# mitschabaude/montgomery

Hardware: AMD Instinct MI355X
Metric: BLS12-377 G1 MSM throughput (higher is better)
Workload: dtype u32

## Files before the change

### montgomery_amd/csrc/msm_internal.h

```cpp
#pragma once
#include "kernel_inst.h"
#include "sort_kernels.h"
#include "tree_kernels.h"
#include "te_kernels.h"
#include "narrow_kernels.h"
#include "host_field.h"
#include "scalar_vec.h"
#include "../../include/msm_hip.h"

#include <algorithm>
#include <cstdarg>
#include <cstdio>
#include <cstring>
#include <atomic>
#include <chrono>
#include <condition_variable>
#include <exception>
#include <functional>
#include <memory>
#include <mutex>
#include <string>
#include <system_error>
#include <thread>
#include <vector>

#ifdef MSM_TUNING
#define MSM_KNOB(var, name, lo) do { if (const char* _e = getenv(name)) var = std::max<long long>((lo), atoll(_e)); } while (0)
#define MSM_KNOB_SET(name) (getenv(name) != nullptr)
#else
#define MSM_KNOB(var, name, lo) do { } while (0)
#define MSM_KNOB_SET(name) false
#endif

namespace msmi {

struct DevBuf {
  void* p = nullptr;
  size_t cap = 0;
};

// ... 112 lines not shown
      std::function<void()> job = std::move(job_);
      job_ = nullptr;
      l.unlock();
      std::exception_ptr e;
      try { job(); } catch (...) { e = std::current_exception(); }
      l.lock();
      err_ = e;
      busy_ = false;
      cv_.notify_all();
    }
  }
  std::mutex mu_;
  std::condition_variable cv_;
  std::function<void()> job_;
  std::exception_ptr err_;
  bool busy_ = false, quit_ = false;
  std::thread th_;
};

}

struct msm_ctx {
  std::unique_ptr<msmi::HelperThread> helper;
  int curve = 0;
  int device = 0;
  hipStream_t stream = nullptr;
  hipEvent_t ev[12] = {};
  hipEvent_t ev_dig[2] = {};
  std::string err;
  int n_cu = 256;

  struct WindowTables {
    int c = 0, K = 0;
    uint64_t lo = 0, n = 0;
    bool in_rows = false;
    msmi::DevBuf buf;
    bool covers(uint64_t l, uint64_t m) const { return K && lo == l && n == m; }
    bool whole_set_pinned() const { return K && in_rows; }
    void clear() { c = K = 0; lo = n = 0; in_rows = false; }
    void drop(msm_ctx* ctx) { clear(); ctx->release(buf); }
  };
  struct PointSet {
    msmi::DevBuf rows;
    uint64_t n = 0;
    bool live = false;
    WindowTables tab;
    const uint32_t* table_rows() const { return (const uint32_t*)(tab.in_rows ? rows.p : tab.buf.p); }
    void release(msm_ctx* ctx) { tab.drop(ctx); ctx->release(rows); *this = PointSet(); }
  };
  std::vector<PointSet> sets = std::vector<PointSet>(1);
  int cur_set = 0;
  PointSet& pts() { return sets[cur_set]; }
  const PointSet& pts() const { return sets[cur_set]; }
  uint32_t* reset_points(uint64_t n) { return reset_points(pts(), n); }
  uint32_t* reset_points(PointSet& s, uint64_t n) {
    s.n = 0;
    s.tab.drop(this);
    cand_n = 0;
    ensure(s.rows, std::max<uint64_t>(n, 1) * row_words() * 4);
    return (uint32_t*)s.rows.p;
  }
  uint64_t cand_lo = 0, cand_n = 0;
  int cand_c = 0;
  uint64_t tables_limit = 0;
  std::vector<void*> allocs;
  std::vector<msm_ctx*> children;
  std::vector<std::unique_ptr<msmi::HelperThread>> fan;

  msmi::DevBuf scal, errflag, misc;
  uint32_t* h_info = nullptr;
  static constexpr int STAGE_THREADS = 4, STAGE_SLOTS = 2;
  static constexpr size_t STAGE_CHUNK = (size_t)16 << 20;
  char* stage_pin = nullptr;
  bool staging_ready = false;
  hipStream_t stage_stream[STAGE_THREADS] = {};
  hipEvent_t stage_ev[STAGE_THREADS][STAGE_SLOTS + 1] = {};
  static constexpr int MAX_PIECES = 6;
  hipEvent_t piece_ev[MAX_PIECES][STAGE_THREADS] = {};
  uint64_t ws_budget = 0;
  uint64_t ws_limit = 0;

  struct Workspace {
    msmi::DevBuf dig, counts, cursor, tail_off, info, slots, block_hist, scan_partial, desc, columns2, rows_sum, bucket_proj, bufA, bufB,
        scratch, columns, partials, part, dig2, idx2, rec, blk_tab2, slots2, dest, rows1, parts, sub;
    hipStream_t stream = nullptr;
    hipStream_t side = nullptr;
    hipEvent_t ev[8] = {};
    uint32_t* h_info = nullptr;
    uint32_t* h_part = nullptr;
    msmi::DevBuf* all[27] = {&dig, &counts, &cursor, &tail_off, &info, &slots, &block_hist, &scan_partial, &desc, &columns2, &rows_sum,
                       &bucket_proj, &bufA, &bufB, &scratch, &columns, &partials, &part, &dig2, &idx2, &rec, &blk_tab2, &slots2, &dest, &rows1,
                       &parts, &sub};
  };
  static constexpr int N_WS = 2;
  Workspace ws[N_WS];

  msm_host::Curve6 hc;
  msm_host::Fe6 k_dev_to_host;
  msm_host::TeCurve6 hte;
  msm_host::Fe6 k_te_to_host;
  bool is_te() const { return curve == MSM_CURVE_ED_ON_BLS12_377; }
  int nl() const { return msmi::curve_info(curve).nl; }
  int nw() const { return msmi::curve_info(curve).nw; }
  size_t coord_bytes() const { return (size_t)nw() * 4; }
  uint64_t row_words() const { return is_te() ? (uint64_t)msm::te::TE_ROW_WORDS : (uint64_t)msm::ROW_WORDS; }
  int sum_words() const { return is_te() ? msmi::TE_SUM_WORDS : msmi::W_SUM_WORDS; }

  void ensure(msmi::DevBuf& b, size_t bytes) {
    if (bytes <= b.cap) return;
    if (b.p) HIPCHK(hipFree(b.p));
    b.p = nullptr;
    b.cap = 0;
    size_t want = bytes + bytes / 16 + 256;
    const hipError_t e = hipMalloc(&b.p, want);
    if (e != hipSuccess) {
      (void)hipGetLastError();
      b.p = nullptr;
      throw msmi::HipFail{e, "hipMalloc(&b.p, want)", __LINE__, __FILE__};
    }
    b.cap = want;
  }
  void release(msmi::DevBuf& b) {
    if (b.p) (void)hipFree(b.p);
    b.p = nullptr;
    b.cap = 0;
  }
};

// ... 22 lines not shown

#define ROWS_TO_PLANES(ctx, ...)                                                                       \
  do {                                                                                                 \
    if ((ctx)->nw() == 8) hipLaunchKernelGGL((k_test_rows_to_planes<8>), __VA_ARGS__);                 \
    else hipLaunchKernelGGL((k_test_rows_to_planes<12>), __VA_ARGS__);                                 \
  } while (0)

namespace msmi {
using namespace msm;

int fail(msm_ctx* ctx, int code, const char* fmt, ...);
int fail_hip(msm_ctx* ctx, const HipFail& f);

inline uint64_t point_lo(const msm_opts* opts) { return opts ? opts->point_lo : 0; }
int check_points(msm_ctx* ctx, uint64_t n, const msm_opts* opts, int code, const char* who, bool empty_ok = true);

#define MSM_CATCH_ALL(ctx)                                                                                  \
  catch (const HipFail& f) { return fail_hip(ctx, f); }                                                     \
  catch (const MsmFail& f) { return fail(ctx, f.code, "%s", f.msg.c_str()); }                               \
  catch (const std::bad_alloc&) { return fail(ctx, MSM_ERR_INTERNAL, "host memory allocation failed"); }    \
  catch (const std::exception& e) { return fail(ctx, MSM_ERR_INTERNAL, "unexpected exception: %s", e.what()); } \
  catch (...) { return fail(ctx, MSM_ERR_INTERNAL, "unexpected exception"); }

int pick_window(bool te, uint64_t n, int glv_max_bits);

struct Plan {
  int c, K, L_log;
  int bits = 0;
  bool fold = false;
  uint32_t L;
  bool no_glv;
  bool strict = false;
  bool lone = false;
  uint32_t b_lo = 0, b_n = 0xFFFFFFFFu;
  uint32_t bt_lo = 0, bt_n = 0xFFFFFFFFu;
  bool tables = false;
  const uint32_t* tab_rows = nullptr;
  uint64_t tab_lo = 0, tab_n = 0;
  bool merged = false;
  int batch = 0;
  BatchScalars batch_sc{};
  struct Narrow {
    int width = 0;
    uint64_t first = 0;
    NarrowFmt fmt{};
    const NarrowBatchScalars* nb = nullptr;
  } nar;
  const uint32_t* idx = nullptr;
};

int make_plan(const msm_ctx* ctx, uint64_t n, const msm_opts* opts, Plan& pl, bool for_tables = false, int narrow_bits = 0);
int pick_window_narrow(bool te, uint64_t n, int bits, bool one_level = false);
int make_run_plan(msm_ctx* ctx, uint64_t n, const msm_opts* opts, bool placed, Plan& pl, bool& tables_wanted, bool note_range = false);

struct GroupStats {
  uint64_t n_pairs = 0;
  uint64_t n_pairs_algo = 0;
  uint64_t max_bucket = 0;
  int rounds = 0;
  float ms_digits = 0, ms_sort = 0, ms_acc = 0, ms_red = 0, ms_r1 = 0;
  GroupStats& operator+=(const GroupStats& o) {
    n_pairs += o.n_pairs;
    n_pairs_algo += o.n_pairs_algo;
    max_bucket = std::max(max_bucket, o.max_bucket);
    rounds += o.rounds;
    ms_digits += o.ms_digits; ms_sort += o.ms_sort; ms_acc += o.ms_acc; ms_red += o.ms_red; ms_r1 += o.ms_r1;
    return *this;
  }
};

struct RoundGeom {
  uint32_t steps, grid;
  uint64_t T;
};

RoundGeom round_geom(const msm_ctx* ctx, uint64_t n_out, bool gather = false, bool lone = false);
void release_workspaces(msm_ctx* ctx);
long double window_bytes(const msm_ctx* ctx, uint64_t n, const Plan& pl);
int windows_per_group(const msm_ctx* ctx, uint64_t n, const Plan& pl);
uint64_t point_pieces(const msm_ctx* ctx, uint64_t n, const Plan& pl);

void words_to_fe6(msm_host::Fe6& r, const uint32_t* w, int nw = 12);
void fe6_to_bytes(uint8_t* out, const msm_host::Fe6& a);
void device_coord_to_wire(const msm_host::Field6& F, const msm_host::Fe6& k_to_host, const uint32_t* w, int nw, uint8_t* out);
void plane_element_to_wire(const msm_ctx* ctx, const uint32_t* planes, uint64_t cap, uint64_t e, uint8_t* out_xy);
void reduce_buckets(msm_ctx* ctx, msm_ctx::Workspace& w, const uint4* fin, uint64_t fin_cap, const uint32_t* off_fin,
// ... 125 lines not shown
      if (turn >= (size_t)S) e = hipEventSynchronize(ctx_->stage_ev[t][slot]);
      if (e != hipSuccess) break;
      memcpy(pin, src_ + off, len);
      e = hipMemcpyAsync(dst_ + off, pin, len, hipMemcpyHostToDevice, ctx_->stage_stream[t % n_streams_]);
      if (e == hipSuccess) e = hipEventRecord(ctx_->stage_ev[t][slot], ctx_->stage_stream[t % n_streams_]);
    }
    mark((int)ends_.size());
    if (e == hipSuccess) e = hipStreamSynchronize(ctx_->stage_stream[t % n_streams_]);
    std::lock_guard<std::mutex> l(mu_);
    rc_[t] = e;
    const float ms = std::chrono::duration<float, std::milli>(std::chrono::steady_clock::now() - t0_).count();
    ms_ = std::max(ms_, ms);
  }
  msm_ctx* ctx_;
  char* dst_;
  const char* src_;
  size_t bytes_;
  std::vector<size_t> ends_;
  std::vector<int> enq_;
  hipError_t rc_[T];
  std::vector<std::thread> th_;
  std::mutex mu_;
  std::condition_variable cv_;
  std::chrono::steady_clock::time_point t0_;
  float ms_ = 0;
  long long n_streams_ = 2;
};

int window_sums_impl(msm_ctx* ctx, const void* scalars, uint64_t n, int on_device, const msm_opts* opts, int k_lo, int k_hi,
                     const Plan& pl, std::vector<uint32_t>& words, msm_result* stats, uint64_t p_off = 0);
int any_window_sums(msm_ctx* ctx, const void* scalars, uint64_t n, int on_device, const msm_opts* opts, int k_lo, int k_hi,
                    const Plan& pl, std::vector<uint32_t>& words, msm_result* stats, const void* const* placed = nullptr);

void run_on_workspaces(msm_ctx* ctx, int n_jobs, bool serial, const std::function<void(int slot, int index)>& job);
void add_group_times(const msm_ctx::Workspace& w, GroupStats& st);
void stats_to_result(const GroupStats& st, msm_result* r);
void add_call_stats(msm_result& tot, const msm_result& r, bool side_by_side = false);
constexpr uint32_t ERR_SCALAR_GE_Q = 4u, ERR_FOLD_DIGIT = 8u;
void check_scalar_flags(msm_ctx* ctx, const Plan& pl, const char* who);

template <class F>
int on_all_devices(msm_ctx* ctx, F f) {
  const int nch = (int)ctx->children.size();
  std::vector<int> rc(nch + 1, MSM_OK);
  std::exception_ptr err;
  for (int i = 0; i < nch; i++) ctx->fan[i]->run([&, i] { rc[i + 1] = f(ctx->children[i]); });
  try { rc[0] = f(ctx); } catch (...) { err = std::current_exception(); }
  for (int i = 0; i < nch; i++) {
    try { ctx->fan[i]->wait(); } catch (...) { if (!err) err = std::current_exception(); }
  }
  if (err) std::rethrow_exception(err);
  for (int i = 0; i <= nch; i++)
    if (rc[i] != MSM_OK) {
      if (i > 0) ctx->err = ctx->children[i - 1]->err;
      return rc[i];
    }
  return MSM_OK;
}

int pick_window_batch(bool te, uint64_t n, uint32_t B, int glv_max_bits);

int narrow_format(msm_ctx* ctx, int32_t width_bytes, int32_t bits, int32_t is_signed, const msm_opts* opts, const char* who,
                  Plan::Narrow& out);
int narrow_scalars_ok(msm_ctx* ctx, const void* scalars, uint64_t n, int on_device, int32_t width_bytes, const char* who);

void translate_payloads(hipStream_t s, const msm_ctx* ctx, uint32_t* slots, uint64_t n_slots, const uint32_t* idx);

// ... 7 lines not shown
```

### montgomery_amd/csrc/msm_pipeline.hip

```cpp
#include "msm_internal.h"

using namespace msm;
using namespace msmi;

namespace {

const uint32_t* group_scalars(const uint32_t* d_scalars_all, uint64_t p_lo, Plan& pl) {
  if (!pl.nar.width) return d_scalars_all + p_lo * 8;
  pl.nar.first += p_lo;
  return d_scalars_all;
}

void run_window_group(msm_ctx* ctx, msm_ctx::Workspace& w, const uint32_t* d_scalars_all, uint64_t p_lo, uint64_t n, const Plan& pl_in,
                      int k_lo, int k_hi, int k_base, uint32_t* h_partials_out, GroupStats& st, uint64_t p_off = 0,
                      GroupDigits* share = nullptr) {
  hipStream_t s = w.stream;
  Plan pl = pl_in;
  const uint32_t* d_scalars = group_scalars(d_scalars_all, p_lo, pl);
  const uint32_t* idx = pl.idx ? pl.idx + p_lo : nullptr;
  p_lo += p_off;
  const int kc = k_hi - k_lo;
  SortOut so;
  HIPCHK(hipEventRecord(w.ev[0], s));
  sort_window_group(ctx, w, d_scalars, n, pl, k_lo, k_hi, st, so, share);
  st.max_bucket = std::max<uint64_t>(st.max_bucket, so.max_bucket);
  if (idx) {
    if (pl.tables || p_off) throw MsmFail{MSM_ERR_INTERNAL, "an indexed group on window tables or over a range of the points"};
    translate_payloads(s, ctx, const_cast<uint32_t*>(so.round1_slots), so.total_slots, idx);
    p_lo = 0;
  }
  HIPCHK(hipEventRecord(w.ev[5], s));
  TreeOut to;
  if (pl.tables) {
    accumulate_window_group(ctx, w, pl, 1, (uint64_t)(k_lo - k_base) * pl.tab_n, so, st, to);
    reduce_buckets(ctx, w, to.fin, to.fin_cap, to.off_fin, to.bucket_proj, pl.L, 1, h_partials_out, pl.merged, pl.c);
    for (int kk = 1; kk < kc; kk++) sum_set_identity(ctx, h_partials_out + (size_t)kk * ctx->sum_words());
  } else {
    accumulate_window_group(ctx, w, pl, kc, p_lo, so, st, to);
    reduce_buckets(ctx, w, to.fin, to.fin_cap, to.off_fin, to.bucket_proj, pl.L, kc, h_partials_out, pl.merged, pl.c);
  }
  add_group_times(w, st);
}

int window_sums_once(msm_ctx* ctx, const void* scalars, uint64_t n, int on_device, const msm_opts* opts, int k_lo, int k_hi,
                     const Plan& pl_in, std::vector<uint32_t>& words, msm_result* stats, uint64_t p_off) {
  Plan pl = pl_in;
  const uint32_t* d_scal = nullptr;
  HIPCHK(hipEventRecord(ctx->ev[8], ctx->stream));
  std::vector<uint64_t> piece_end;
  if (!on_device && pipelines_host_scalars(n)) {
    piece_end = pipelined_piece_ends(n);
    ctx->ensure(ctx->scal, n * 32);
  }
  std::unique_ptr<PieceUpload> pipe;
  if (piece_end.empty()) stage_scalars(ctx, scalars, n, on_device, &d_scal);
  HIPCHK(hipEventRecord(ctx->ev[9], ctx->stream));
  GroupStats st;
  const int pw = ctx->sum_words();
  words.assign((size_t)(k_hi - k_lo) * pw, 0);
  if (ctx->ws_limit) {
    ctx->ws_budget = ctx->ws_limit;
  } else if (n >= (1ull << 22)) {
    size_t free_b = 0, total_b = 0;
    HIPCHK(hipMemGetInfo(&free_b, &total_b));
    uint64_t held = 0;
    for (auto& w : ctx->ws)
      for (DevBuf* b : w.all) held += b->cap;
    ctx->ws_budget = (uint64_t)((free_b + held) * 0.85L);
  }
  int wpg = std::min(windows_per_group(ctx, n, pl), 128);
  {
    const uint64_t entries = ctx->is_te() ? n : 2 * n;
    const bool fits_lds = ((size_t)pl.L * 4 <= 128 * 1024);
    if (pl.c - 1 > (int)RX_FINE_BITS && (!fits_lds || entries >= one_level_entry_limit(ctx->is_te()))) wpg = std::min(wpg, 16);
    if (pl.tables) wpg = std::min(wpg, 16);
  }
  const int nwin = k_hi - k_lo;
  int want_groups = (nwin >= 2 && (n >= (1ull << 22) || (pl.tables && n >= (ctx->is_te() ? 1ull << 20 : 1ull << 21)))) ? 2 : 1;
  MSM_KNOB(want_groups, "MSM_GROUPS", 1);
  wpg = std::max(1, std::min(wpg, (nwin + want_groups - 1) / want_groups));
  struct Group {
    int ka, kb;
    uint64_t p_lo, p_n;
    int piece;
  };
  std::vector<Group> groups;
  uint64_t pieces = 1;
  if (nwin == 1 && want_groups == 1 && !ctx->is_te() && n >= (1ull << 24) && !MSM_KNOB_SET("MSM_GROUPS")) pieces = 2;
  pieces = std::max(pieces, point_pieces(ctx, n, pl));
  if (!piece_end.empty() && point_pieces(ctx, n, pl) > 1) {
    piece_end.clear();
    stage_scalars(ctx, scalars, n, on_device, &d_scal);
  }
  if (!piece_end.empty()) {
    ctx->ensure(ctx->scal, n * 32);
    d_scal = (const uint32_t*)ctx->scal.p;
    uint64_t lo = 0;
    for (size_t q = 0; q < piece_end.size(); q++) {
      const uint64_t cnt = piece_end[q] - lo;
      const int g = (nwin >= 2 && cnt >= (1ull << 22)) ? 2 : 1;
      const int per = std::max(1, std::min(wpg, (nwin + g - 1) / g));
      for (int k = k_lo; k < k_hi; k += per) groups.push_back({k, std::min(k_hi, k + per), lo, cnt, (int)q});
      lo = piece_end[q];
    }
  } else if (pieces > 1) {
    for (int k = k_lo; k < k_hi; k++)
      for (uint64_t q = 0; q < pieces; q++) {
        const uint64_t lo = n * q / pieces, hi = n * (q + 1) / pieces;
        groups.push_back({k, k + 1, lo, hi - lo, -1});
      }
  } else {
    for (int k = k_lo; k < k_hi; k += wpg) groups.push_back({k, std::min(k_hi, k + wpg), 0, n, -1});
  }
  bool split_points = false;
  for (const Group& g : groups) split_points |= g.p_n != n;
  if (pl.tables && (split_points || n != pl.tab_n || p_off != pl.tab_lo)) pl.tables = false;
  std::vector<std::vector<uint32_t>> split_part((split_points || pl.tables) ? groups.size() : 0);
  HIPCHK(hipMemsetAsync(ctx->errflag.p, 0, 4, ctx->stream));
  HIPCHK(hipStreamSynchronize(ctx->stream));
  if (!piece_end.empty()) {
    std::vector<size_t> ends;
    for (uint64_t e : piece_end) ends.push_back((size_t)e * 32);
    pipe.reset(new PieceUpload(ctx, ctx->scal.p, scalars, n * 32, ends));
  }
  GroupDigits share;
  if (groups.size() == 2 && !ctx->is_te() && groups[0].piece < 0 && groups[1].piece < 0 &&
      groups[0].p_lo == groups[1].p_lo && groups[0].p_n == groups[1].p_n && groups[0].kb == groups[1].ka &&
      groups[1].kb - groups[0].ka <= 16) {
    share.produce = true;
    share.ready = ctx->ev_dig[1];
    SortOut none;
    GroupStats gs;
    HIPCHK(hipEventRecord(ctx->ev_dig[0], ctx->ws[0].stream));
    Plan pd = pl;
    const uint32_t* d_grp = group_scalars(d_scal, groups[0].p_lo, pd);
    sort_window_group(ctx, ctx->ws[0], d_grp, groups[0].p_n, pd, groups[0].ka, groups[1].kb, gs, none, &share);
    share.produce = false;
  }
  GroupStats sts[msm_ctx::N_WS];
  run_on_workspaces(ctx, (int)groups.size(), opts && opts->serial, [&](int slot, int gi) {
    const int ka = groups[gi].ka, kb = groups[gi].kb;
    std::vector<uint32_t> part((size_t)(kb - ka) * pw);
    Plan pg = pl;
    pg.lone = (groups.size() == 1 && (kb - ka == 1 || pl.tables)) || (opts && opts->serial);
    if (groups[gi].piece >= 0) pipe->wait_piece(groups[gi].piece, ctx->ws[slot].stream);
    run_window_group(ctx, ctx->ws[slot], d_scal, groups[gi].p_lo, groups[gi].p_n, pg, ka, kb, k_lo, part.data(), sts[slot], p_off,
                     share.valid ? &share : nullptr);
    if (split_points || pl.tables) split_part[gi] = part;
    else memcpy(&words[(size_t)(ka - k_lo) * pw], part.data(), part.size() * 4);
  });
  check_scalar_flags(ctx, pl, "msm_run_narrow");
  float upload_ms = -1;
  if (pipe) upload_ms = pipe->finish();
  if (pl.tables) {
    std::vector<const uint32_t*> firsts;
    for (const auto& part : split_part)
      if (!part.empty()) firsts.push_back(part.data());
    sum_slots(ctx, firsts, words.data());
    for (int k = k_lo + 1; k < k_hi; k++) sum_set_identity(ctx, &words[(size_t)(k - k_lo) * pw]);
  } else if (split_points) {
    for (int k = k_lo; k < k_hi; k++) {
      std::vector<const uint32_t*> ranges;
      for (size_t gi = 0; gi < groups.size(); gi++)
        if (groups[gi].ka <= k && k < groups[gi].kb && !split_part[gi].empty())
          ranges.push_back(split_part[gi].data() + (size_t)(k - groups[gi].ka) * pw);
      sum_slots(ctx, ranges, &words[(size_t)(k - k_lo) * pw]);
    }
  }
  if (share.valid) {
    float ms;
    HIPCHK(hipEventElapsedTime(&ms, ctx->ev_dig[0], ctx->ev_dig[1]));
    st.ms_digits += ms;
  }
  for (const GroupStats& g : sts) st += g;
  HIPCHK(hipEventRecord(ctx->ev[10], ctx->stream));
  HIPCHK(hipStreamSynchronize(ctx->stream));
  if (stats) {
    float ms;
    HIPCHK(hipEventElapsedTime(&ms, ctx->ev[8], ctx->ev[9]));
    stats->phase_ms[MSM_T_UPLOAD] = upload_ms >= 0 ? upload_ms : ms;
    HIPCHK(hipEventElapsedTime(&ms, ctx->ev[8], ctx->ev[10]));
    stats->phase_ms[MSM_T_TOTAL] = ms;
    stats_to_result(st, stats);
    stats->c = pl.c;
    stats->K = pl.K;
    stats->tables = pl.tables ? 1 : 0;
  }
  return MSM_OK;
}

}

namespace msmi {

void run_on_workspaces(msm_ctx* ctx, int n_jobs, bool serial, const std::function<void(int slot, int index)>& job) {
  std::atomic<int> next{0};
  auto worker = [&](int slot) {
    HIPCHK(hipSetDevice(ctx->device));
    for (int i; (i = next.fetch_add(1)) < n_jobs;) job(slot, i);
  };
  const int nthreads = serial ? 1 : std::min<int>(msm_ctx::N_WS, n_jobs);
  std::exception_ptr err;
  if (nthreads > 1) ctx->helper->run([&] { worker(1); });
  try { worker(0); } catch (...) { err = std::current_exception(); }
  if (nthreads > 1) {
    try { ctx->helper->wait(); } catch (...) { if (!err) err = std::current_exception(); }
  }
  if (err) {
    for (auto& w : ctx->ws) (void)hipStreamSynchronize(w.stream);
    std::rethrow_exception(err);
  }
}

void add_group_times(const msm_ctx::Workspace& w, GroupStats& st) {
  float ms;
  HIPCHK(hipEventElapsedTime(&ms, w.ev[0], w.ev[1])); st.ms_digits += ms;
  HIPCHK(hipEventElapsedTime(&ms, w.ev[1], w.ev[2])); st.ms_sort += ms;
  HIPCHK(hipEventElapsedTime(&ms, w.ev[5], w.ev[3])); st.ms_acc += ms;
  HIPCHK(hipEventElapsedTime(&ms, w.ev[5], w.ev[6])); st.ms_r1 += ms;
  HIPCHK(hipEventElapsedTime(&ms, w.ev[3], w.ev[4])); st.ms_red += ms;
}

void stats_to_result(const GroupStats& st, msm_result* r) {
  r->phase_ms[MSM_T_DIGITS] = st.ms_digits;
  r->phase_ms[MSM_T_SORT] = st.ms_sort;
  r->phase_ms[MSM_T_ACCUMULATE] = st.ms_acc;
  r->phase_ms[MSM_T_ACC_ROUND1] = st.ms_r1;
  r->phase_ms[MSM_T_REDUCE] = st.ms_red;
  r->n_pairs = st.n_pairs;
  r->n_pairs_algo = st.n_pairs_algo;
  r->max_bucket = st.max_bucket;
// ... 129 lines not shown
```

### montgomery_amd/csrc/msm_tree.hip

```cpp
#include "msm_internal.h"

using namespace msm;
using namespace msmi;

namespace msmi {

void accumulate_window_group(msm_ctx* ctx, msm_ctx::Workspace& w, const Plan& pl, int kc, uint64_t row_off, const SortOut& so,
                             GroupStats& st, TreeOut& to) {
  hipStream_t s = w.stream;
  const bool lone = pl.lone;
  const bool te = ctx->is_te();
  const uint32_t L = pl.L;
  const uint64_t nb = (uint64_t)kc * L;
  const size_t elem_bytes = te ? 128 : 96;
  const uint32_t logG = so.logG;
  const int RT = so.RT;
  const uint64_t total_slots = so.total_slots;
  const uint32_t max_bucket = so.max_bucket;
  const uint32_t* round1_slots = so.round1_slots;
  const uint32_t* round1_dest = so.round1_dest;
  const uint64_t rec_y_off = so.rec_y_off;
  const bool chunked = so.chunked;

  uint32_t FINISH_MAX = pl.c >= 18 ? 64 : 32;
// ... 9 lines not shown
           (((cap_elems + (1u << r_stop) - 1) >> r_stop) > FINISH_MAX || w.h_info[3 + r_stop + 1] >= tail_min_pairs))
      r_stop++;
  }
  uint64_t capA = 1, capB = 1;
  {
    int which = 0;
    uint64_t cnt = total_slots;
    for (uint32_t r = 1; r <= logG; r++) {
      cnt /= 2;
      if (r == 1 && chunked) continue;
      (which ? capB : capA) = std::max<uint64_t>(which ? capB : capA, cnt);
      which ^= 1;
    }
    for (int r = 1; r <= r_stop; r++) {
      cnt = w.h_info[3 + r];
      (which ? capB : capA) = std::max<uint64_t>(which ? capB : capA, cnt);
      which ^= 1;
    }
  }
  const size_t tree_slack = (size_t)2 * 257 * 512 * 16 + 4096;
  ctx->ensure(w.bufA, capA * elem_bytes + tree_slack);
  ctx->ensure(w.bufB, capB * elem_bytes + tree_slack);
  uint4* buf[2] = {(uint4*)w.bufA.p, (uint4*)w.bufB.p};
  uint64_t cap[2] = {capA, capB};
  int cur = 0;
  uint64_t n_in = total_slots;
  int round = 0;
  const uint4* fin = buf[0];
  uint64_t fin_cap = cap[0];
  const uint32_t* off_fin = (const uint32_t*)w.tail_off.p;
  if (total_slots > 0) {
    for (uint32_t r = 1; r <= logG; r++) {
      uint64_t n_out = n_in / 2;
      RoundGeom g = round_geom(ctx, n_out, r == 1 || (r == 2 && chunked) || te, lone);
      const uint64_t sstride = g.T;
      if (!te) ctx->ensure(w.scratch, (size_t)g.steps * NL * sstride * 4);
      BatchArgs a{};
      a.points = (pl.tables ? pl.tab_rows : (const uint32_t*)ctx->pts().rows.p) + row_off * ctx->row_words();
      a.slots = r == 1 ? round1_slots : (const uint32_t*)w.slots.p;
      a.dest = r == 1 ? round1_dest : nullptr;
      a.in = buf[cur ^ 1];
      a.in_cap = cap[cur ^ 1];
      a.out = buf[cur];
      a.out_cap = cap[cur];
      a.scratch = (uint32_t*)w.scratch.p;
      a.sstride = sstride;
      a.n_out = n_out;
      a.steps = g.steps;
      const bool rows_out = r == 1 && chunked, rows_in = r == 2 && chunked;
      a.y_off = 4 * ctx->nw();
      if (rows_out) a.out_rows = (uint32_t*)w.rows1.p;
      if (rows_in) { a.points = (const uint32_t*)w.rows1.p; a.slots = nullptr; }
      if (rows_out) a.out_y_off = rec_y_off;
      if (rows_in && ctx->nw() == 12) a.y_off = rec_y_off;
      if (r == 1 || rows_in) {
        if (te) hipLaunchKernelGGL(te::k_te_add<MODE_GATHER>, dim3(g.grid), dim3(256), 0, s, a);
        else W_LAUNCH_MODE(ctx, k_batch_add, MODE_GATHER, dim3(g.grid), dim3(256), 0, s, a);
        if (r == 1) HIPCHK(hipEventRecord(w.ev[6], s));
      } else {
        if (te) hipLaunchKernelGGL(te::k_te_add<MODE_REGULAR>, dim3(g.grid), dim3(256), 0, s, a);
        else W_LAUNCH_MODE(ctx, k_batch_add, MODE_REGULAR, dim3(g.grid), dim3(256), 0, s, a);
      }
      st.n_pairs += n_out;
      n_in = n_out;
      round++;
      if (rows_out) continue;
      fin = buf[cur];
// ... 68 lines not shown
```

### montgomery_amd/csrc/msm_abi.hip

```cpp
#include "msm_internal.h"
#include <chrono>

using namespace msm;
using namespace msmi;

extern "C" {

uint32_t msm_abi_version(void) { return MSM_ABI_VERSION; }
uint32_t msm_abi_struct_bytes(int which) { return which == 0 ? (uint32_t)sizeof(msm_opts) : which == 1 ? (uint32_t)sizeof(msm_result) : 0u; }

int msm_ctx_create(msm_ctx** out, int curve, int device) {
  if (!out) return MSM_ERR_ARG;
  *out = nullptr;
  if (!curve_info_or_null(curve)) return MSM_ERR_ARG;
  int ndev = 0;
  if (hipGetDeviceCount(&ndev) != hipSuccess || ndev <= 0 || device < 0 || device >= ndev) return MSM_ERR_NO_DEVICE;
  msm_ctx* ctx = new (std::nothrow) msm_ctx();
  if (!ctx) return MSM_ERR_INTERNAL;
  ctx->curve = curve;
  ctx->device = device;
  try {
    ctx->helper.reset(new HelperThread());
    HIPCHK(hipSetDevice(device));
    hipDeviceProp_t prop;
    HIPCHK(hipGetDeviceProperties(&prop, device));
    ctx->n_cu = prop.multiProcessorCount > 0 ? prop.multiProcessorCount : 256;
    HIPCHK(hipStreamCreateWithFlags(&ctx->stream, hipStreamNonBlocking));
    for (auto& e : ctx->ev) HIPCHK(hipEventCreate(&e));
    for (auto& e : ctx->ev_dig) HIPCHK(hipEventCreate(&e));
    HIPCHK(hipHostMalloc((void**)&ctx->h_info, 64 * 4, hipHostMallocDefault));
    for (auto& w : ctx->ws) {
      HIPCHK(hipStreamCreateWithFlags(&w.stream, hipStreamNonBlocking));
      HIPCHK(hipStreamCreateWithFlags(&w.side, hipStreamNonBlocking));
      for (auto& e : w.ev) HIPCHK(hipEventCreate(&e));
      HIPCHK(hipHostMalloc((void**)&w.h_info, 64 * 4, hipHostMallocDefault));
      HIPCHK(hipHostMalloc((void**)&w.h_part, 128 * 20 * W_SUM_WORDS * 4, hipHostMallocDefault));
    }
    size_t free_b = 0, total_b = 0;
    HIPCHK(hipMemGetInfo(&free_b, &total_b));
    ctx->ws_budget = (uint64_t)(free_b * 0.55);
    ctx->tables_limit = (uint64_t)(total_b * 0.10);
    ctx->ensure(ctx->errflag, 16);
    sort_kernel_attributes();
  } catch (const HipFail& f) {
    fprintf(stderr, "msm_ctx_create: HIP error %s at line %d\n", hipGetErrorString(f.e), f.line);
    msm_ctx_destroy(ctx);
    return MSM_ERR_HIP;
  } catch (...) {
    msm_ctx_destroy(ctx);
    return MSM_ERR_INTERNAL;
  }
  ctx->hc.F.init(curve == MSM_CURVE_ED_ON_BLS12_377 ? Fp377::PW : curve_info(curve).pw);
  ctx->k_dev_to_host = ctx->hc.F.pow2(2 * ctx->hc.F.radix_bits() - 30 * ctx->nl());
  {
    uint32_t pw[12] = {0};
    for (int i = 0; i < 8; i++) pw[i] = Fp253::PW[i];
    ctx->hte.init(pw, 3021);
    ctx->k_te_to_host = ctx->hte.F.pow2(2 * ctx->hte.F.radix_bits() - 270);
  }
  *out = ctx;
  return MSM_OK;
}

void msm_ctx_destroy(msm_ctx* ctx) {
  if (!ctx) return;
  ctx->fan.clear();
  for (msm_ctx* c : ctx->children) msm_ctx_destroy(c);
  ctx->children.clear();
  (void)hipSetDevice(ctx->device);
  for (void* p : ctx->allocs) (void)hipFree(p);
  ctx->allocs.clear();
  if (ctx->stream) (void)hipStreamSynchronize(ctx->stream);
  for (auto& s : ctx->sets) s.release(ctx);
  for (DevBuf* b : {&ctx->scal, &ctx->errflag, &ctx->misc}) ctx->release(*b);
// ... 431 lines not shown
```

### montgomery_amd/csrc/msm_tables.hip

```cpp
#include "msm_internal.h"

using namespace msm;
using namespace msmi;

namespace msmi {

static uint64_t table_bytes(const msm_ctx* ctx, uint64_t n, int K) {
  return (uint64_t)K * std::max<uint64_t>(n, 1) * ctx->row_words() * 4;
}

static void build_tables(msm_ctx* ctx, const Plan& pl, uint64_t lo, uint64_t n) {
  msm_ctx::PointSet& ps = ctx->pts();
  msm_ctx::WindowTables& t = ps.tab;
  const bool whole = lo == 0 && n == ps.n;
  const uint64_t row_words = ctx->row_words();
  const uint64_t bytes = table_bytes(ctx, n, pl.K);
  HIPCHK(hipStreamSynchronize(ctx->stream));
  auto ensure_or_retry = [&](DevBuf& b) {
    try {
      ctx->ensure(b, bytes);
    } catch (const HipFail& f) {
      if (f.e != hipErrorOutOfMemory) throw;
      (void)hipGetLastError();
      release_workspaces(ctx);
      ctx->release(ctx->scal);
      ctx->ensure(b, bytes);
    }
  };
  uint32_t* rows = nullptr;
  if (whole) {
    t.drop(ctx);
    if (ps.rows.cap < bytes) {
      DevBuf big;
      ensure_or_retry(big);
      HIPCHK(hipMemcpyAsync(big.p, ps.rows.p, n * row_words * 4, hipMemcpyDeviceToDevice, ctx->stream));
      HIPCHK(hipStreamSynchronize(ctx->stream));
      ctx->release(ps.rows);
      ps.rows = big;
    }
    rows = (uint32_t*)ps.rows.p;
  } else {
    t.clear();
    ensure_or_retry(t.buf);
    rows = (uint32_t*)t.buf.p;
    HIPCHK(hipMemcpyAsync(rows, (const uint32_t*)ps.rows.p + lo * row_words, n * row_words * 4, hipMemcpyDeviceToDevice, ctx->stream));
  }
  const uint32_t grid = (uint32_t)((n + 255) / 256);
  for (int k = 1; k < pl.K; k++) {
    uint32_t* out = rows + (uint64_t)k * n * row_words;
    const uint32_t* in = rows + (uint64_t)(k - 1) * n * row_words;
    if (ctx->is_te()) hipLaunchKernelGGL(te::k_te_table_next, dim3(grid), dim3(256), 0, ctx->stream, out, in, n, pl.c);
    else W_LAUNCH(ctx, k_table_next, dim3(grid), dim3(256), 0, ctx->stream, out, in, n, pl.c);
  }
  HIPCHK(hipStreamSynchronize(ctx->stream));
  HIPCHK(hipGetLastError());
  t.c = pl.c;
  t.K = pl.K;
  t.lo = lo;
  t.n = n;
  t.in_rows = whole;
}

static bool tables_eligible(const msm_ctx* ctx, uint64_t n, const msm_opts* opts, bool placed) {
  if (placed || (opts && (opts->no_tables || opts->bucket_shards > 1))) return false;
  if (!ctx->children.empty()) return false;
  return point_lo(opts) + n <= ctx->pts().n && n >= 4096;
}
static bool whole_set(const msm_ctx* ctx, uint64_t n, const msm_opts* opts) { return n == ctx->pts().n && point_lo(opts) == 0; }
static bool whole_set_tables_stay(const msm_ctx* ctx, uint64_t n, const msm_opts* opts) {
  return ctx->pts().tab.whole_set_pinned() && !whole_set(ctx, n, opts);
}
static bool tables_fit(const msm_ctx* ctx, uint64_t n, int K) {
  return table_bytes(ctx, n, K) <= ctx->tables_limit && (uint64_t)K * (ctx->is_te() ? n : 2 * n) < (1ull << 31);
}
static bool buildable(const msm_ctx* ctx, uint64_t n, const msm_opts* opts, const Plan& pl) {
  return tables_eligible(ctx, n, opts, false) && pl.K >= 2 && tables_fit(ctx, n, pl.K);
}

static bool plan_suits_tables(const Plan& pl) {
  if (pl.K < 2) return false;
  const int top_bits = pl.fold ? pl.c + 1 : pl.bits - (pl.K - 1) * pl.c;
  return top_bits >= pl.c - 3;
}

static bool builds_now(const msm_ctx* ctx, uint64_t n, const msm_opts* opts, int c) {
  return whole_set(ctx, n, opts) || (ctx->cand_n == n && ctx->cand_lo == point_lo(opts) && ctx->cand_c == c);
}

int make_run_plan(msm_ctx* ctx, uint64_t n, const msm_opts* opts, bool placed, Plan& pl, bool& tables_wanted, bool note_range) {
  tables_wanted = false;
  if (tables_eligible(ctx, n, opts, placed)) {
    const msm_ctx::WindowTables& t = ctx->pts().tab;
    msm_opts o;
    if (opts) o = *opts; else memset(&o, 0, sizeof o);
    const int asked = o.c;
    Plan pt, pd;
    o.c = asked ? asked : t.c;
    if (t.covers(point_lo(opts), n) && make_plan(ctx, n, &o, pt) == MSM_OK && pt.c == t.c && pt.K == t.K &&
        (asked ? asked == t.c : make_plan(ctx, n, opts, pd, true) == MSM_OK && pd.c == t.c)) {
      pl = pt;
      tables_wanted = true;
      return MSM_OK;
    }
    o.c = 0;
    if (!o.no_glv && make_plan(ctx, n, &o, pt, true) == MSM_OK && (asked == 0 || asked == pt.c) && plan_suits_tables(pt) &&
        buildable(ctx, n, opts, pt) && !whole_set_tables_stay(ctx, n, opts)) {
      const bool build_now = builds_now(ctx, n, opts, pt.c);
      if (note_range && !whole_set(ctx, n, opts)) {
        ctx->cand_lo = point_lo(opts);
        ctx->cand_n = n;
        ctx->cand_c = pt.c;
      }
      pl = pt;
      tables_wanted = build_now || !note_range;
      return MSM_OK;
    }
  }
  return make_plan(ctx, n, opts, pl);
}

bool use_window_tables(msm_ctx* ctx, uint64_t n, const msm_opts* opts, Plan& pl) {
  const msm_ctx::PointSet& ps = ctx->pts();
  const uint64_t lo = point_lo(opts);
  if (!(tables_eligible(ctx, n, opts, false) && ps.tab.covers(lo, n) && ps.tab.c == pl.c && ps.tab.K == pl.K)) {
    if (!buildable(ctx, n, opts, pl) || whole_set_tables_stay(ctx, n, opts)) return false;
    build_tables(ctx, pl, lo, n);
  }
  pl.tab_rows = ps.table_rows();
  pl.tab_lo = ps.tab.lo;
  pl.tab_n = ps.tab.n;
  return true;
}

}

extern "C" {

int msm_precompute(msm_ctx* ctx, uint64_t n, const msm_opts* opts) {
  if (!ctx) return MSM_ERR_ARG;
  if (int rc = check_points(ctx, n, opts, MSM_ERR_ARG, "msm_precompute", false)) return rc;
  Plan pl;
  if (make_plan(ctx, n, opts, pl, true)) return fail(ctx, MSM_ERR_ARG, "msm_precompute: bad window size");
  try {
    HIPCHK(hipSetDevice(ctx->device));
    if (whole_set_tables_stay(ctx, n, opts) && buildable(ctx, n, opts, pl)) ctx->pts().tab.drop(ctx);
    (void)use_window_tables(ctx, n, opts, pl);
    return MSM_OK;
  } MSM_CATCH_ALL(ctx)
}

int msm_tables_info(const msm_ctx* ctx, int32_t* c_out, int32_t* K_out, uint64_t* bytes_out) {
  if (!ctx) return MSM_ERR_ARG;
  const msm_ctx::WindowTables& t = ctx->pts().tab;
  if (c_out) *c_out = t.c;
  if (K_out) *K_out = t.K;
  if (bytes_out) *bytes_out = t.K ? table_bytes(ctx, t.n, t.K) : 0;
  return MSM_OK;
}

int msm_tables_range(const msm_ctx* ctx, uint64_t* point_lo_out, uint64_t* n_out) {
  if (!ctx) return MSM_ERR_ARG;
  if (point_lo_out) *point_lo_out = ctx->pts().tab.lo;
  if (n_out) *n_out = ctx->pts().tab.n;
  return MSM_OK;
}

int msm_set_tables_limit(msm_ctx* ctx, uint64_t bytes) {
  if (!ctx) return MSM_ERR_ARG;
  ctx->tables_limit = bytes;
  for (msm_ctx* c : ctx->children) c->tables_limit = bytes;
  return MSM_OK;
}

}
```

Baseline: 515.7 million.

## Rendezvous the two window-group streams before tree accumulation starts

Adds a host-side GroupSync rendezvous so the two window-group workers exchange stream events after sorting. Under the default IN_STEP policy each stream waits for the other's sort-done event before its tree phase, so both groups' tree kernels run together rather than one group's sort overlapping the other's tree. A STAGGERED option instead makes group 1 wait for group 0's round-1 add and gives group 0 a lone geometry for round 1. This trades sort/tree overlap for less contention between the two streams' tree kernels, and adds host thread blocking.

```diff
diff --git a/montgomery_amd/csrc/group_sync.h b/montgomery_amd/csrc/group_sync.h
--- /dev/null
+++ b/montgomery_amd/csrc/group_sync.h
@@ -0,0 +1,68 @@
+#pragma once
+#include <condition_variable>
+#include <mutex>
+
+namespace msmi {
+
+template <class Token>
+class GroupSync {
+ public:
+  static constexpr int PARTIES = 2, POINTS = 2;
+
+  void reset() {
+    std::lock_guard<std::mutex> l(mu_);
+    for (int p = 0; p < PARTIES; p++) {
+      gone_[p] = false;
+      for (int i = 0; i < POINTS; i++) posted_[p][i] = false;
+    }
+  }
+  void post(int me, int pt, Token t) {
+    {
+      std::lock_guard<std::mutex> l(mu_);
+      tok_[me][pt] = t;
+      posted_[me][pt] = true;
+    }
+    cv_.notify_all();
+  }
+  bool await(int who, int pt, Token* out) {
+    std::unique_lock<std::mutex> l(mu_);
+    cv_.wait(l, [&] { return posted_[who][pt] || gone_[who]; });
+    if (!posted_[who][pt]) return false;
+    *out = tok_[who][pt];
+    return true;
+  }
+  bool arrive(int me, int pt, Token t, Token* other) {
+    post(me, pt, t);
+    return await(1 - me, pt, other);
+  }
+  void depart(int me) {
+    {
+      std::lock_guard<std::mutex> l(mu_);
+      gone_[me] = true;
+    }
+    cv_.notify_all();
+  }
+
+  class Party {
+   public:
+    Party(GroupSync* sync, int me) : sync_(sync), me_(me) {}
+    Party(const Party&) = delete;
+    Party& operator=(const Party&) = delete;
+    ~Party() {
+      if (sync_) sync_->depart(me_);
+    }
+
+   private:
+    GroupSync* sync_;
+    int me_;
+  };
+
+ private:
+  std::mutex mu_;
+  std::condition_variable cv_;
+  Token tok_[PARTIES][POINTS] = {};
+  bool posted_[PARTIES][POINTS] = {};
+  bool gone_[PARTIES] = {};
+};
+
+}
diff --git a/montgomery_amd/csrc/msm_internal.h b/montgomery_amd/csrc/msm_internal.h
--- a/montgomery_amd/csrc/msm_internal.h
+++ b/montgomery_amd/csrc/msm_internal.h
@@ -6,6 +6,7 @@
 #include "narrow_kernels.h"
 #include "host_field.h"
 #include "scalar_vec.h"
+#include "group_sync.h"
 #include "../../include/msm_hip.h"
 
 #include <algorithm>
@@ -246,6 +247,7 @@
   };
   static constexpr int N_WS = 2;
   Workspace ws[N_WS];
+  msmi::GroupSync<hipEvent_t> group_sync;
 
   msm_host::Curve6 hc;
   msm_host::Fe6 k_dev_to_host;
@@ -334,6 +336,7 @@
   bool no_glv;
   bool strict = false;
   bool lone = false;
+  bool lone_r1 = false;
   uint32_t b_lo = 0, b_n = 0xFFFFFFFFu;
   uint32_t bt_lo = 0, bt_n = 0xFFFFFFFFu;
   bool tables = false;
@@ -545,7 +548,9 @@
 int any_window_sums(msm_ctx* ctx, const void* scalars, uint64_t n, int on_device, const msm_opts* opts, int k_lo, int k_hi,
                     const Plan& pl, std::vector<uint32_t>& words, msm_result* stats, const void* const* placed = nullptr);
 
-void run_on_workspaces(msm_ctx* ctx, int n_jobs, bool serial, const std::function<void(int slot, int index)>& job);
+void run_on_workspaces(msm_ctx* ctx, int n_jobs, bool serial, const std::function<void(int slot, int index)>& job,
+                       GroupSync<hipEvent_t>* sync = nullptr);
+enum class TreeStart { FREE = 0, IN_STEP = 1, STAGGERED = 2 };
 void add_group_times(const msm_ctx::Workspace& w, GroupStats& st);
 void stats_to_result(const GroupStats& st, msm_result* r);
 void add_call_stats(msm_result& tot, const msm_result& r, bool side_by_side = false);
diff --git a/montgomery_amd/csrc/msm_pipeline.hip b/montgomery_amd/csrc/msm_pipeline.hip
--- a/montgomery_amd/csrc/msm_pipeline.hip
+++ b/montgomery_amd/csrc/msm_pipeline.hip
@@ -13,7 +13,8 @@
 
 void run_window_group(msm_ctx* ctx, msm_ctx::Workspace& w, const uint32_t* d_scalars_all, uint64_t p_lo, uint64_t n, const Plan& pl_in,
                       int k_lo, int k_hi, int k_base, uint32_t* h_partials_out, GroupStats& st, uint64_t p_off = 0,
-                      GroupDigits* share = nullptr) {
+                      GroupDigits* share = nullptr, GroupSync<hipEvent_t>* sync = nullptr, int party = 0,
+                      TreeStart start = TreeStart::FREE) {
   hipStream_t s = w.stream;
   Plan pl = pl_in;
   const uint32_t* d_scalars = group_scalars(d_scalars_all, p_lo, pl);
@@ -24,6 +25,11 @@
   HIPCHK(hipEventRecord(w.ev[0], s));
   sort_window_group(ctx, w, d_scalars, n, pl, k_lo, k_hi, st, so, share);
   st.max_bucket = std::max<uint64_t>(st.max_bucket, so.max_bucket);
+  if (sync && start != TreeStart::FREE) {
+    hipEvent_t other;
+    if (sync->arrive(party, 0, w.ev[2], &other)) HIPCHK(hipStreamWaitEvent(s, other, 0));
+    if (start == TreeStart::STAGGERED && party == 1 && sync->await(0, 1, &other)) HIPCHK(hipStreamWaitEvent(s, other, 0));
+  }
   if (idx) {
     if (pl.tables || p_off) throw MsmFail{MSM_ERR_INTERNAL, "an indexed group on window tables or over a range of the points"};
     translate_payloads(s, ctx, const_cast<uint32_t*>(so.round1_slots), so.total_slots, idx);
@@ -33,10 +39,12 @@
   TreeOut to;
   if (pl.tables) {
     accumulate_window_group(ctx, w, pl, 1, (uint64_t)(k_lo - k_base) * pl.tab_n, so, st, to);
+    if (sync && start == TreeStart::STAGGERED && party == 0) sync->post(0, 1, w.ev[6]);
     reduce_buckets(ctx, w, to.fin, to.fin_cap, to.off_fin, to.bucket_proj, pl.L, 1, h_partials_out, pl.merged, pl.c);
     for (int kk = 1; kk < kc; kk++) sum_set_identity(ctx, h_partials_out + (size_t)kk * ctx->sum_words());
   } else {
     accumulate_window_group(ctx, w, pl, kc, p_lo, so, st, to);
+    if (sync && start == TreeStart::STAGGERED && party == 0) sync->post(0, 1, w.ev[6]);
     reduce_buckets(ctx, w, to.fin, to.fin_cap, to.off_fin, to.bucket_proj, pl.L, kc, h_partials_out, pl.merged, pl.c);
   }
   add_group_times(w, st);
@@ -78,6 +86,12 @@
   const int nwin = k_hi - k_lo;
   int want_groups = (nwin >= 2 && (n >= (1ull << 22) || (pl.tables && n >= (ctx->is_te() ? 1ull << 20 : 1ull << 21)))) ? 2 : 1;
   MSM_KNOB(want_groups, "MSM_GROUPS", 1);
+  TreeStart start_policy = TreeStart::IN_STEP;
+  {
+    int v = (int)start_policy;
+    MSM_KNOB(v, "MSM_TREE_START", 0);
+    start_policy = (TreeStart)std::min(v, (int)TreeStart::STAGGERED);
+  }
   wpg = std::max(1, std::min(wpg, (nwin + want_groups - 1) / want_groups));
   struct Group {
     int ka, kb;
@@ -137,18 +151,24 @@
     sort_window_group(ctx, ctx->ws[0], d_grp, groups[0].p_n, pd, groups[0].ka, groups[1].kb, gs, none, &share);
     share.produce = false;
   }
+  const bool serial = opts && opts->serial;
+  TreeStart start = TreeStart::FREE;
+  if (groups.size() == 2 && !serial && !split_points && groups[0].piece < 0 && groups[1].piece < 0) start = start_policy;
+  GroupSync<hipEvent_t>* sync = start != TreeStart::FREE ? &ctx->group_sync : nullptr;
+  if (sync) sync->reset();
   GroupStats sts[msm_ctx::N_WS];
-  run_on_workspaces(ctx, (int)groups.size(), opts && opts->serial, [&](int slot, int gi) {
+  run_on_workspaces(ctx, (int)groups.size(), serial, [&](int slot, int gi) {
     const int ka = groups[gi].ka, kb = groups[gi].kb;
     std::vector<uint32_t> part((size_t)(kb - ka) * pw);
     Plan pg = pl;
-    pg.lone = (groups.size() == 1 && (kb - ka == 1 || pl.tables)) || (opts && opts->serial);
+    pg.lone = (groups.size() == 1 && (kb - ka == 1 || pl.tables)) || serial;
+    pg.lone_r1 = start == TreeStart::STAGGERED && slot == 0;
     if (groups[gi].piece >= 0) pipe->wait_piece(groups[gi].piece, ctx->ws[slot].stream);
     run_window_group(ctx, ctx->ws[slot], d_scal, groups[gi].p_lo, groups[gi].p_n, pg, ka, kb, k_lo, part.data(), sts[slot], p_off,
-                     share.valid ? &share : nullptr);
+                     share.valid ? &share : nullptr, sync, slot, start);
     if (split_points || pl.tables) split_part[gi] = part;
     else memcpy(&words[(size_t)(ka - k_lo) * pw], part.data(), part.size() * 4);
-  });
+  }, sync);
   check_scalar_flags(ctx, pl, "msm_run_narrow");
   float upload_ms = -1;
   if (pipe) upload_ms = pipe->finish();
@@ -193,10 +213,14 @@
 
 namespace msmi {
 
-void run_on_workspaces(msm_ctx* ctx, int n_jobs, bool serial, const std::function<void(int slot, int index)>& job) {
+void run_on_workspaces(msm_ctx* ctx, int n_jobs, bool serial, const std::function<void(int slot, int index)>& job,
+                       GroupSync<hipEvent_t>* sync) {
+  if (sync && (serial || n_jobs != msm_ctx::N_WS)) throw MsmFail{MSM_ERR_INTERNAL, "a rendezvous call needs one job per worker"};
   std::atomic<int> next{0};
   auto worker = [&](int slot) {
+    GroupSync<hipEvent_t>::Party party(sync, slot);
     HIPCHK(hipSetDevice(ctx->device));
+    if (sync) return job(slot, slot);
     for (int i; (i = next.fetch_add(1)) < n_jobs;) job(slot, i);
   };
   const int nthreads = serial ? 1 : std::min<int>(msm_ctx::N_WS, n_jobs);
diff --git a/montgomery_amd/csrc/msm_tree.hip b/montgomery_amd/csrc/msm_tree.hip
--- a/montgomery_amd/csrc/msm_tree.hip
+++ b/montgomery_amd/csrc/msm_tree.hip
@@ -65,7 +65,7 @@
   if (total_slots > 0) {
     for (uint32_t r = 1; r <= logG; r++) {
       uint64_t n_out = n_in / 2;
-      RoundGeom g = round_geom(ctx, n_out, r == 1 || (r == 2 && chunked) || te, lone);
+      RoundGeom g = round_geom(ctx, n_out, r == 1 || (r == 2 && chunked) || te, lone || (r == 1 && pl.lone_r1));
       const uint64_t sstride = g.T;
       if (!te) ctx->ensure(w.scratch, (size_t)g.steps * NL * sstride * 4);
       BatchArgs a{};
```

Result: no change. 512.2 million (-0.7%).

## Store only per-group window tables and combine group results with Horner doubling

Applied to the files above, without the earlier changes.

Precomputed window tables now hold only as many shifted copies as one window group needs (T = ceil(K/groups)) instead of all K windows. Every group reuses the same table offset, and the group partial sums are combined by Horner-style doubling by c*wpg bits. This halves table memory, which together with a doubled tables_limit lets tables fit for larger n or more points. The cost is extra host-side doublings and a coupling between table count and group split.

```diff
diff --git a/montgomery_amd/csrc/msm_abi.hip b/montgomery_amd/csrc/msm_abi.hip
--- a/montgomery_amd/csrc/msm_abi.hip
+++ b/montgomery_amd/csrc/msm_abi.hip
@@ -39,7 +39,7 @@
     size_t free_b = 0, total_b = 0;
     HIPCHK(hipMemGetInfo(&free_b, &total_b));
     ctx->ws_budget = (uint64_t)(free_b * 0.55);
-    ctx->tables_limit = (uint64_t)(total_b * 0.10);
+    ctx->tables_limit = (uint64_t)(total_b * 0.20);
     ctx->ensure(ctx->errflag, 16);
     sort_kernel_attributes();
   } catch (const HipFail& f) {
diff --git a/montgomery_amd/csrc/msm_internal.h b/montgomery_amd/csrc/msm_internal.h
--- a/montgomery_amd/csrc/msm_internal.h
+++ b/montgomery_amd/csrc/msm_internal.h
@@ -184,12 +184,13 @@
 
   struct WindowTables {
     int c = 0, K = 0;
+    int T = 0;
     uint64_t lo = 0, n = 0;
     bool in_rows = false;
     msmi::DevBuf buf;
     bool covers(uint64_t l, uint64_t m) const { return K && lo == l && n == m; }
     bool whole_set_pinned() const { return K && in_rows; }
-    void clear() { c = K = 0; lo = n = 0; in_rows = false; }
+    void clear() { T = 0; c = K = 0; lo = n = 0; in_rows = false; }
     void drop(msm_ctx* ctx) { clear(); ctx->release(buf); }
   };
   struct PointSet {
@@ -339,6 +340,7 @@
   bool tables = false;
   const uint32_t* tab_rows = nullptr;
   uint64_t tab_lo = 0, tab_n = 0;
+  int tab_T = 0;
   bool merged = false;
   int batch = 0;
   BatchScalars batch_sc{};
@@ -354,6 +356,10 @@
 int make_plan(const msm_ctx* ctx, uint64_t n, const msm_opts* opts, Plan& pl, bool for_tables = false, int narrow_bits = 0);
 int pick_window_narrow(bool te, uint64_t n, int bits, bool one_level = false);
 int make_run_plan(msm_ctx* ctx, uint64_t n, const msm_opts* opts, bool placed, Plan& pl, bool& tables_wanted, bool note_range = false);
+
+inline int window_groups_wanted(bool te, uint64_t n, bool tables, int nwin) {
+  return (nwin >= 2 && (n >= (1ull << 22) || (tables && n >= (te ? 1ull << 20 : 1ull << 21)))) ? 2 : 1;
+}
 
 struct GroupStats {
   uint64_t n_pairs = 0;
diff --git a/montgomery_amd/csrc/msm_pipeline.hip b/montgomery_amd/csrc/msm_pipeline.hip
--- a/montgomery_amd/csrc/msm_pipeline.hip
+++ b/montgomery_amd/csrc/msm_pipeline.hip
@@ -12,8 +12,7 @@
 }
 
 void run_window_group(msm_ctx* ctx, msm_ctx::Workspace& w, const uint32_t* d_scalars_all, uint64_t p_lo, uint64_t n, const Plan& pl_in,
-                      int k_lo, int k_hi, int k_base, uint32_t* h_partials_out, GroupStats& st, uint64_t p_off = 0,
-                      GroupDigits* share = nullptr) {
+                      int k_lo, int k_hi, uint32_t* h_partials_out, GroupStats& st, uint64_t p_off = 0, GroupDigits* share = nullptr) {
   hipStream_t s = w.stream;
   Plan pl = pl_in;
   const uint32_t* d_scalars = group_scalars(d_scalars_all, p_lo, pl);
@@ -32,7 +31,8 @@
   HIPCHK(hipEventRecord(w.ev[5], s));
   TreeOut to;
   if (pl.tables) {
-    accumulate_window_group(ctx, w, pl, 1, (uint64_t)(k_lo - k_base) * pl.tab_n, so, st, to);
+    if (kc > pl.tab_T) throw MsmFail{MSM_ERR_INTERNAL, "a window group on window tables with more windows than tables"};
+    accumulate_window_group(ctx, w, pl, 1, 0, so, st, to);
     reduce_buckets(ctx, w, to.fin, to.fin_cap, to.off_fin, to.bucket_proj, pl.L, 1, h_partials_out, pl.merged, pl.c);
     for (int kk = 1; kk < kc; kk++) sum_set_identity(ctx, h_partials_out + (size_t)kk * ctx->sum_words());
   } else {
@@ -76,9 +76,10 @@
     if (pl.tables) wpg = std::min(wpg, 16);
   }
   const int nwin = k_hi - k_lo;
-  int want_groups = (nwin >= 2 && (n >= (1ull << 22) || (pl.tables && n >= (ctx->is_te() ? 1ull << 20 : 1ull << 21)))) ? 2 : 1;
+  int want_groups = window_groups_wanted(ctx->is_te(), n, pl.tables, nwin);
   MSM_KNOB(want_groups, "MSM_GROUPS", 1);
   wpg = std::max(1, std::min(wpg, (nwin + want_groups - 1) / want_groups));
+  if (pl.tables) wpg = std::max(1, std::min(wpg, pl.tab_T));
   struct Group {
     int ka, kb;
     uint64_t p_lo, p_n;
@@ -144,7 +145,7 @@
     Plan pg = pl;
     pg.lone = (groups.size() == 1 && (kb - ka == 1 || pl.tables)) || (opts && opts->serial);
     if (groups[gi].piece >= 0) pipe->wait_piece(groups[gi].piece, ctx->ws[slot].stream);
-    run_window_group(ctx, ctx->ws[slot], d_scal, groups[gi].p_lo, groups[gi].p_n, pg, ka, kb, k_lo, part.data(), sts[slot], p_off,
+    run_window_group(ctx, ctx->ws[slot], d_scal, groups[gi].p_lo, groups[gi].p_n, pg, ka, kb, part.data(), sts[slot], p_off,
                      share.valid ? &share : nullptr);
     if (split_points || pl.tables) split_part[gi] = part;
     else memcpy(&words[(size_t)(ka - k_lo) * pw], part.data(), part.size() * 4);
@@ -153,10 +154,9 @@
   float upload_ms = -1;
   if (pipe) upload_ms = pipe->finish();
   if (pl.tables) {
-    std::vector<const uint32_t*> firsts;
-    for (const auto& part : split_part)
-      if (!part.empty()) firsts.push_back(part.data());
-    sum_slots(ctx, firsts, words.data());
+    std::vector<uint32_t> firsts(groups.size() * (size_t)pw);
+    for (size_t gi = 0; gi < groups.size(); gi++) memcpy(&firsts[gi * pw], split_part[gi].data(), (size_t)pw * 4);
+    sums_horner(ctx, firsts.data(), (int)groups.size(), pl.c * wpg, words.data());
     for (int k = k_lo + 1; k < k_hi; k++) sum_set_identity(ctx, &words[(size_t)(k - k_lo) * pw]);
   } else if (split_points) {
     for (int k = k_lo; k < k_hi; k++) {
diff --git a/montgomery_amd/csrc/msm_tables.hip b/montgomery_amd/csrc/msm_tables.hip
--- a/montgomery_amd/csrc/msm_tables.hip
+++ b/montgomery_amd/csrc/msm_tables.hip
@@ -5,8 +5,12 @@
 
 namespace msmi {
 
-static uint64_t table_bytes(const msm_ctx* ctx, uint64_t n, int K) {
-  return (uint64_t)K * std::max<uint64_t>(n, 1) * ctx->row_words() * 4;
+static int tables_held(const msm_ctx* ctx, uint64_t n, int K) {
+  const int groups = window_groups_wanted(ctx->is_te(), n, true, K);
+  return (K + groups - 1) / groups;
+}
+static uint64_t table_bytes(const msm_ctx* ctx, uint64_t n, int T) {
+  return (uint64_t)T * std::max<uint64_t>(n, 1) * ctx->row_words() * 4;
 }
 
 static void build_tables(msm_ctx* ctx, const Plan& pl, uint64_t lo, uint64_t n) {
@@ -14,7 +18,8 @@
   msm_ctx::WindowTables& t = ps.tab;
   const bool whole = lo == 0 && n == ps.n;
   const uint64_t row_words = ctx->row_words();
-  const uint64_t bytes = table_bytes(ctx, n, pl.K);
+  const int T = tables_held(ctx, n, pl.K);
+  const uint64_t bytes = table_bytes(ctx, n, T);
   HIPCHK(hipStreamSynchronize(ctx->stream));
   auto ensure_or_retry = [&](DevBuf& b) {
     try {
@@ -46,7 +51,7 @@
     HIPCHK(hipMemcpyAsync(rows, (const uint32_t*)ps.rows.p + lo * row_words, n * row_words * 4, hipMemcpyDeviceToDevice, ctx->stream));
   }
   const uint32_t grid = (uint32_t)((n + 255) / 256);
-  for (int k = 1; k < pl.K; k++) {
+  for (int k = 1; k < T; k++) {
     uint32_t* out = rows + (uint64_t)k * n * row_words;
     const uint32_t* in = rows + (uint64_t)(k - 1) * n * row_words;
     if (ctx->is_te()) hipLaunchKernelGGL(te::k_te_table_next, dim3(grid), dim3(256), 0, ctx->stream, out, in, n, pl.c);
@@ -59,6 +64,7 @@
   t.lo = lo;
   t.n = n;
   t.in_rows = whole;
+  t.T = T;
 }
 
 static bool tables_eligible(const msm_ctx* ctx, uint64_t n, const msm_opts* opts, bool placed) {
@@ -71,7 +77,8 @@
   return ctx->pts().tab.whole_set_pinned() && !whole_set(ctx, n, opts);
 }
 static bool tables_fit(const msm_ctx* ctx, uint64_t n, int K) {
-  return table_bytes(ctx, n, K) <= ctx->tables_limit && (uint64_t)K * (ctx->is_te() ? n : 2 * n) < (1ull << 31);
+  const int T = tables_held(ctx, n, K);
+  return table_bytes(ctx, n, T) <= ctx->tables_limit && (uint64_t)T * (ctx->is_te() ? n : 2 * n) < (1ull << 31);
 }
 static bool buildable(const msm_ctx* ctx, uint64_t n, const msm_opts* opts, const Plan& pl) {
   return tables_eligible(ctx, n, opts, false) && pl.K >= 2 && tables_fit(ctx, n, pl.K);
@@ -129,6 +136,7 @@
   pl.tab_rows = ps.table_rows();
   pl.tab_lo = ps.tab.lo;
   pl.tab_n = ps.tab.n;
+  pl.tab_T = ps.tab.T;
   return true;
 }
 
@@ -154,7 +162,7 @@
   const msm_ctx::WindowTables& t = ctx->pts().tab;
   if (c_out) *c_out = t.c;
   if (K_out) *K_out = t.K;
-  if (bytes_out) *bytes_out = t.K ? table_bytes(ctx, t.n, t.K) : 0;
+  if (bytes_out) *bytes_out = t.K ? table_bytes(ctx, t.n, t.T) : 0;
   return MSM_OK;
 }
 
```

Result: faster. 514.8 million before, 527.3 million after (median of 6 runs) (+2.4%).
